# indrajeetadityaroy9/vit-inductive-bias-distillation

Hardware: AMD Instinct MI355X
Metric: distillation images/sec (BASD loss fwd+bwd+grad all-reduce), DeiT-S<-ResNet-50 @ bs256/GPU (higher is better)
Workload: dtype f32; 1 GPU; cfg2 DeiT-S<-ResNet-50 224x224; per_gpu_batch=256, global_batch=256, input_dtype=float32, layout=strided (CLS-sliced / channel-major views), backward=True, grad_allreduce_bytes=88202672, grad_allreduce=none at world size 1 (bucket packed, nothing to exchange), rank_readback=auto, readback_deferred_steps=1756, selector=basd_selector_chain mode 0, parallelism=dp1

## Files before the change

include/basd_hip.h:

```cpp
#ifndef BASD_HIP_H
#define BASD_HIP_H

#include <stdint.h>

#ifdef __cplusplus
extern "C" {
#endif

#ifndef __HIP_PLATFORM_AMD__
typedef struct ihipStream_t* hipStream_t;
#endif

#define BASD_OK 0
#define BASD_EINVAL (-1)
#define BASD_EUNSUPPORTED (-2)
#define BASD_DTYPE_F32 0
#define BASD_DTYPE_BF16 1


int basd_gemm_nt(const void* a, int a_dtype, long a_sb, long a_sn, long a_sd, int a_rows_per_batch,
                 long a_batch_stride, const float* b, long ldb, long b_batch_stride, int M, int N, int K, int batch,
                 float* c, long ldc, long c_batch_stride, float scale, const float* bias, float beta,
                 float* colsum_part, float* col_mean, hipStream_t stream);

// ... 144 lines not shown
                         const float* omega, const int* tap0, const int* tap1, const float* lam, const int* range0,
                         const int* range1, float* mu, float* tr_s, float* a_prime, hipStream_t stream);

int basd_teacher_center(const void* const* tok_ptrs, int dtype, const float* mix, int L, long sb, long sn, long sd,
                        int B, int n, int D, const int* g0, const int* g1, const float* glam, const float* omega_t,
                        float* mu, float* tc, hipStream_t stream);
int basd_teacher_center_multi(const void* const* tok_ptrs, int dtype, const float* mix, int L, int G, long sb, long sn,
                              long sd, int B, int n, int D, const int* g0, const int* g1, const float* glam,
                              const float* omega_t, float* mu, float* tc, hipStream_t stream);
long basd_teacher_center_stream_scratch_floats(int G, int B, int n, int D);
int basd_teacher_center_stream(const void* const* tok_ptrs, int dtype, const float* mix, int L, int G, long sb, long sn,
                               long sd, int B, int n, int D, const int* g0, const int* g1, const float* glam,
                               const float* omega_t, float* mu, float* tc, float* scratch, hipStream_t stream);

int basd_gram_f64(const float* p, long p_batch_stride, int n, int D, int batch, double* g, long g_batch_stride,
                  hipStream_t stream);

int basd_gram_f64_split(const float* p, long p_batch_stride, int n, int D, int batch, int splits, double* slabs,
                        double* g, hipStream_t stream);

int basd_chol_f64(const double* g, long g_batch_stride, int n, int batch, double* l, long l_batch_stride,
                  hipStream_t stream);

int basd_stack_product(const double* la, const double* lb, long l_batch_stride, int n, int batch, int lb_period,
                       float* w, long w_batch_stride, hipStream_t stream);

int basd_procrustes_finalize(const float* w, long w_batch_stride, const float* sigma, int n, int n_s, int batch,
                             int t_period ,
                             const double* gb, long g_batch_stride, const float* omega, const int* tap0,
                             const int* tap1, const float* lam, const float* tr_s_part, int tr_slabs, float* tr_s,
                             float* tr_t, float* nuc, float* loss, float* k_prime, hipStream_t stream);

int basd_student_grad(const void* x, int dtype, long sb, long sn, int B, int n_s, int n_t, int D, const float* omega,
                      const float* mu, const float* h, const int* tap0, const int* tap1, const float* lam,
                      const float* scale_ptr, float scale_const, float* dx, const float* tnorm2, float* gomega,
                      hipStream_t stream);

int basd_student_project_multi(const void* const* x_ptrs, int dtype, long sb, long sn, int E, int B, int n_s, int n_t,
                               int D, int ptrs_16B_aligned, const float* omega, long omega_e_stride, const int* tap0,
                               const int* tap1, const float* lam, const int* range0, const int* range1, float* mu,
                               float* tr_s, float* a_prime, hipStream_t stream);
int basd_student_grad_multi(const void* const* x_ptrs, int dtype, long sb, long sn, int E, int B, int n_s, int n_t,
                            int D, const float* omega, long omega_e_stride, const float* mu, const float* h,
                            const int* tap0, const int* tap1, const float* lam, const float* scale_ptr,
                            float scale_const, float* dx, const float* tnorm2, float* gomega, hipStream_t stream);
int basd_student_grad_fused(const void* const* x_ptrs, int dtype, long sb, long sn, int E, int B, int n_s, int n_t,
// ... 8 lines not shown
    long s_dtype, s_sb, s_sn, s_aligned;
    const void* const* tok_ptrs;
    long t_dtype, t_sb, t_sn, t_sd;
    const void* const* attn_ptrs;
    long a_dtype, a_sb, a_sh, a_sq, a_sk;
    const float* mix;
    long E, L, G, B, n_s, n_t, d_s, d_t, H, A, has_cls, n_a, n, max_sweeps;
    const int* atap0; const int* atap1; const float* alam;
    const int* tap0; const int* tap1; const float* lam; const int* range0; const int* range1;
    const int* g0; const int* g1; const float* glam;
    float* omega; float* omega_t; float* raw; float* mu_t; float* tc; float* mu_s; float* tr_part; float* tr_s;
    float* a_prime;
    double* g_all; double* l_all;
    float* W; float* sigma; int* jflags; int* sweeps;
    float* tr_t; float* nuc; float* loss_b; float* k_prime;
    float* h; float* dx; const float* grad_layers;
    double* g_slabs; long g_splits;
    const float* uw_ce; float* uw_out;
    void* jac_ws;
    float* w_stack; float* sigma_u;
} BasdProcrustesArgs;
int basd_procrustes_forward_fused(const BasdProcrustesArgs* args, hipStream_t stream);
int basd_procrustes_tuning(int transposed_cores);

int basd_stack_product_t(const double* la, const double* lb, long l_batch_stride, int n, int batch, int lb_period,
                         float* w, long w_batch_stride, hipStream_t stream);
int basd_kprime_from_transposed(const float* w, long w_batch_stride, const float* sigma, int n, int batch,
                                const double* lb, long l_batch_stride, int lb_period, float* z, long z_batch_stride,
                                float* k_prime, hipStream_t stream);
int basd_ustack_stash(const float* wc, long wc_batch_stride, int n, int batch, float* w_stack, long w_stack_stride,
                      hipStream_t stream);
int basd_ustack_from_transposed(const float* x, long x_batch_stride, const float* sigma, int n, int batch,
                                float* w_stack, long w_stack_stride, float* scratch, long scratch_batch_stride,
                                float* sigma_u, int max_sweeps, int* jflags, hipStream_t stream);

int basd_scale_unless_one(float* x, long count, const float* num, const float* den, hipStream_t stream);

int basd_cross_entropy(const void* logits, int dtype, long ld, int B, int C, const long* labels, const float* probs,
                       long pld, float label_smoothing, long ignore_index, float* row_loss, float* dlogits,
                       hipStream_t stream);


int basd_event_create(void** out);
int basd_event_destroy(void* event);
int basd_stream_wait_event(hipStream_t stream, void* event);
int basd_event_record(void* event, hipStream_t stream);
// ... 84 lines not shown
```

vit-inductive-bias-distillation_amd/basd_amd/_lib.py:

```python
from __future__ import annotations

import ctypes as C
import os
import threading

_HERE = os.path.dirname(os.path.abspath(__file__))
LIB_PATH = os.path.join(_HERE, "libbasd_hip.so")

vp, i32, i64, f32, f64 = C.c_void_p, C.c_int, C.c_long, C.c_float, C.c_double

SIGNATURES = {
    "basd_gemm_nt": [vp, i32, i64, i64, i64, i32, i64, vp, i64, i64, i32, i32, i32, i32, vp, i64, i64, f32, vp, f32,
                     vp, vp, vp],
    "basd_gemm_tn_splits": [i32],
    "basd_gemm_tn": [vp, vp, i32, i64, i64, i64, i64, i64, i64, i64, i64, i32, i32, i32, i32, i32, vp, vp, i32, vp,
                     vp, i64, i64, f32, vp],
    "basd_colmean_parts": [i32],
    "basd_colmean": [vp, i32, i64, i64, i64, i32, i64, i32, i32, i32, i32, vp, vp, vp],
    "basd_colmean_multi": [vp, i32, i64, i64, i64, i32, i32, i32, i32, i32, vp, vp, i32, vp],
    "basd_syrk_splits": [i32, i32, i32],
    "basd_syrk_multi": [vp, i32, i64, i64, i64, i32, i32, i32, i32, vp, vp, i32, vp, vp, i64, i32, vp, i32, i32, vp],
    "basd_jacobi_workspace_ints": [i32, i32],
    "basd_jacobi_twopass_workspace_bytes": [i32, i32, i32],
    "basd_jacobi_stacked_twopass": [vp, i64, i32, i32, vp, i32, i32, f32, vp, vp, vp],
# ... 16 lines not shown
    "basd_tridiag_eigenvalues": [vp, vp, i32, i32, vp, vp],
    "basd_tridiag_apply_q": [vp, vp, i32, i32, i32, vp, vp, i32, i32, vp],
    "basd_tridiag_shifted_solve": [vp, vp, vp, i32, i32, i32, i32, vp, vp, vp],
    "basd_tridiag_mp_rank": [vp, vp, i32, i32, f64, i32, vp, vp, vp, vp, vp],
    "basd_tridiag_mp_rank_rank1": [vp, vp, vp, i32, i32, f64, f64, i32, vp, vp, vp, vp],
    "basd_tridiag_eigenvectors": [vp, vp, vp, vp, vp, i32, i32, i32, vp, vp, i32, vp],
    "basd_mp_rank": [vp, i32, i32, f64, i32, vp, vp, vp],
    "basd_grassmann_distance": [vp, i32, vp, vp, i32, vp, i32, vp, vp, vp],
    "basd_grassmann_distance_padded": [vp, i32, i32, vp, vp, i32, vp, i32, vp, vp],
    "basd_selector_tail": [vp] * 10 + [i32, i32, i32, i32] + [vp] * 14 + [vp],
    "basd_sqrt_clamp": [vp, vp, i64, vp],
    "basd_gram_finish": [vp, vp, i32, i32, i64, vp, vp, vp],
    "basd_cross_entropy": [vp, i32, i64, i32, i32, vp, vp, i64, f32, i64, vp, vp, vp],
    "basd_token_weights": [vp, i32, vp, i32, i64, i64, i64, i64, i32, i32, i32, i32, i32, i32, i32, vp, vp, vp, vp,
                           vp, vp, vp, vp, vp, vp],
    "basd_student_project": [vp, i32, i64, i64, i32, i32, i32, i32, vp, vp, vp, vp, vp, vp, vp, vp, vp, vp],
    "basd_teacher_center": [vp, i32, vp, i32, i64, i64, i64, i32, i32, i32, vp, vp, vp, vp, vp, vp, vp],
    "basd_teacher_center_multi": [vp, i32, vp, i32, i32, i64, i64, i64, i32, i32, i32, vp, vp, vp, vp, vp, vp, vp],
    "basd_teacher_center_stream_scratch_floats": [i32, i32, i32, i32],
    "basd_teacher_center_stream": [vp, i32, vp, i32, i32, i64, i64, i64, i32, i32, i32, vp, vp, vp, vp, vp, vp, vp, vp],
    "basd_gram_f64": [vp, i64, i32, i32, i32, vp, i64, vp],
    "basd_gram_f64_split": [vp, i64, i32, i32, i32, i32, vp, vp, vp],
    "basd_chol_f64": [vp, i64, i32, i32, vp, i64, vp],
    "basd_stack_product": [vp, vp, i64, i32, i32, i32, vp, i64, vp],
    "basd_procrustes_finalize": [vp, i64, vp, i32, i32, i32, i32, vp, i64, vp, vp, vp, vp, vp, i32, vp, vp, vp, vp,
                                 vp, vp],
    "basd_student_project_multi": [vp, i32, i64, i64, i32, i32, i32, i32, i32, i32, vp, i64, vp, vp, vp, vp, vp, vp,
                                   vp, vp, vp],
    "basd_student_grad_multi": [vp, i32, i64, i64, i32, i32, i32, i32, i32, vp, i64, vp, vp, vp, vp, vp, vp, f32, vp,
                                vp, vp, vp],
    "basd_student_grad_fused": [vp, i32, i64, i64, i32, i32, i32, i32, i32, i32, vp, i64, vp, vp, vp, vp, vp, vp, vp,
                                f32, vp, vp],
    "basd_procrustes_forward_fused": [vp, vp],
    "basd_procrustes_tuning": [i32],
    "basd_jacobi_plain4_fits": [i32],
    "basd_stack_product_t": [vp, vp, i64, i32, i32, i32, vp, i64, vp],
    "basd_kprime_from_transposed": [vp, i64, vp, i32, i32, vp, i64, i32, vp, i64, vp, vp],
    "basd_ustack_stash": [vp, i64, i32, i32, vp, i64, vp],
    "basd_ustack_from_transposed": [vp, i64, vp, i32, i32, vp, i64, vp, i64, vp, i32, vp, vp],
    "basd_resample_tokens": [vp, i32, i64, i64, i64, i32, i32, i32, i32, vp, vp, vp, vp, vp],
    "basd_resample_tokens_adjoint": [vp, i32, i32, i32, i32, vp, vp, vp, vp, vp, vp, vp],
    "basd_student_grad": [vp, i32, i64, i64, i32, i32, i32, i32, vp, vp, vp, vp, vp, vp, vp, f32, vp, vp, vp, vp],
    "basd_teacher_factor": [vp, i64, vp, i32, i32, i32, vp, vp, i64, vp, vp, vp, vp, vp, vp, vp, vp, vp],
    "basd_teacher_factor_tiled": [vp, i64, vp, i32, i32, i32, vp, vp, i64, vp, vp, vp, vp, vp, vp, vp, vp, vp, vp],
    "basd_mix_grad_tokens": [vp, vp, i32, i32, i64, i64, i64, i32, i32, i32, i32, vp, vp, vp, vp, vp],
    "basd_mix_grad_tokens_scratch_floats": [i32, i32, i32, i32],
    "basd_mix_grad_tokens_onepass": [vp, vp, i32, i32, i64, i64, i64, i32, i32, i32, i32, vp, vp, vp, vp, vp, vp],
    "basd_token_weight_bwd": [vp, vp, i32, i32, i32, i32, vp, vp, vp, vp, vp, vp, i32, i32, i64, i64, i64, i64, i32,
                              i32, i32, vp, vp, vp],
    "basd_build_angle_stack": [vp, i32, vp, i32, vp, vp],
    "basd_grassmann_distance_bwd": [vp, vp, i32, vp, vp, i32, vp, vp, i32, vp, vp],
    "basd_eigvec_k2": [vp, vp, i32, i32, i32, vp, vp],
    "basd_selector_chain": [vp],
    "basd_rank_certificate": [vp, vp, i32, i32, f64, vp, vp, vp],
    "basd_rank_certificate_scratch_bytes": [i32],
    "basd_debug_fill_lds": [C.c_uint, vp],
    "basd_selector_chain_tail": [vp, i32, i32],
# ... 105 lines not shown
```

vit-inductive-bias-distillation_amd/basd_amd/ops.py:

```python
from __future__ import annotations

from dataclasses import dataclass
from functools import lru_cache

import torch

from . import _lib

import os

F32, BF16 = 0, 1
MAX_SWEEPS = 20
TWO_PASS_SVD = True
TRANSPOSED_MIX_GRAD = True
TWO_PASS_LOG_LIMIT = 16 << 30
EIG_SOLVER = os.environ.get("BASD_EIG_SOLVER", "tridiag")
if os.environ.get("BASD_GEMM_SPLIT") in ("0", "1"):
    _lib.call("basd_gemm_tuning", int(os.environ["BASD_GEMM_SPLIT"]))
if os.environ.get("BASD_JACOBI_ORDERING") in ("0", "1"):
    _lib.call("basd_jacobi_ordering", int(os.environ["BASD_JACOBI_ORDERING"]))


def _stream() -> int:
    return torch._C._cuda_getCurrentRawStream(torch._C._cuda_getDevice())


def _dtype_code(t: torch.Tensor) -> int:
    if t.dtype == torch.float32:
        return F32
    if t.dtype == torch.bfloat16:
        return BF16
    raise TypeError(f"unsupported dtype {t.dtype}")


def as_supported(t: torch.Tensor) -> torch.Tensor:
    if t.dtype in (torch.float32, torch.bfloat16):
        return t
# ... 472 lines not shown
        self.E, self.L, self.B, self.n_s, self.d_s, self.n_t, self.d_t = E, L, B, n_s, d_s, n_t, d_t
        n_a = A - (1 if has_cls else 0)
        n = min(n_s, n_t)
        self.n, self.n_a = n, n_a
        self.tp = taps(n_t, n_s, dev) if n_t < n_s else None
        self.gt = taps(n_t, n_s, dev) if n_t > n_s else None
        self.atp = taps(n_a, n_s, dev)
        G = self.G = 1 if L == 1 else E
        f32 = dict(device=dev, dtype=torch.float32)
        slabs = (d_s + 31) // 32
        EB, GB = E * B, G * B
        self.need_bwd, self.need_mix_grad, self.want_dx, self.want_uw = need_bwd, need_mix_grad, want_dx, want_uw
        self.kept_sizes = [G * B * n_s, E * B * d_s, EB * n * d_s, EB * n * n if need_bwd else 0, 4 * EB,
                           (4 + 2 * E) if want_uw else 0]
        self.kept_padded = [(c + 63) // 64 * 64 for c in self.kept_sizes]
        self.kept_total = sum(self.kept_padded)
        g_splits = 1
        if GB < 1024 and d_t >= 512:
            g_splits = max(1, min(1024 // GB, d_t // 256, 16))
        self.g_splits = g_splits
        self.g_all = torch.empty((EB + GB + (g_splits * GB if g_splits > 1 else 0), n, n), device=dev, dtype=torch.float64)
        self.l_all = torch.empty((EB + GB, n, n), device=dev, dtype=torch.float64)
        self.W = torch.empty((EB, n, 2 * n), **f32)
        self.tc = torch.empty((G, B, n, d_t), **f32)
        sizes = [GB * n, GB * d_t, EB * slabs, EB * n]
        padded = [(c + 63) // 64 * 64 for c in sizes]
        self.omega_t, self.mu_t, self.tr_part, self.sigma = (
            piece[:c] for piece, c in zip(torch.split(torch.empty((sum(padded),), **f32), padded), sizes))
        self.ints = torch.empty((_lib.query("basd_jacobi_workspace_ints", EB, MAX_SWEEPS) + EB,), device=dev,
                                dtype=torch.int32)
        self.sweeps = self.ints[-EB:] if want_sweeps else None
        transposed_mix = bool(need_mix_grad and need_bwd and _lib.query("basd_jacobi_plain4_fits", n)
                              and (EB >= 128 or TRANSPOSED_MIX_GRAD == "force") and TRANSPOSED_MIX_GRAD)
        jac_bytes = _lib.query("basd_jacobi_twopass_workspace_bytes", n, EB, MAX_SWEEPS) \
            if TWO_PASS_SVD and not transposed_mix else 0
        if jac_bytes > TWO_PASS_LOG_LIMIT or (jac_bytes > (256 << 20)
                                              and jac_bytes > torch.cuda.mem_get_info(dev)[0] // 2):
            jac_bytes = 0
        self.jac_ws = torch.empty((jac_bytes // 8 + 1,), device=dev, dtype=torch.int64) if jac_bytes > 0 else None
        self.h = torch.empty((E, B, n, d_s), **f32) if want_dx else None
        self.w_stack = None
        self.sigma_u = None
        if transposed_mix:
            self.w_stack = torch.empty((EB, n, 2 * n), **f32)
            self.sigma_u = torch.empty((EB, n), **f32)
        self.host_ptrs = (ctypes.c_void_p * E)()

        a = self.args = _lib.ProcrustesArgs()
        a.student_host_ptrs = ctypes.cast(self.host_ptrs, ctypes.c_void_p)
        (a.E, a.L, a.G, a.B, a.n_s, a.n_t, a.d_s, a.d_t, a.H, a.A, a.has_cls, a.n_a, a.n, a.max_sweeps) = \
            E, L, G, B, n_s, n_t, d_s, d_t, H, A, int(has_cls), n_a, n, MAX_SWEEPS
        if self.atp:
            a.atap0, a.atap1, a.alam = self.atp.tap0.data_ptr(), self.atp.tap1.data_ptr(), self.atp.lam.data_ptr()
        if self.tp:
            a.tap0, a.tap1, a.lam = self.tp.tap0.data_ptr(), self.tp.tap1.data_ptr(), self.tp.lam.data_ptr()
            a.range0, a.range1 = self.tp.range0.data_ptr(), self.tp.range1.data_ptr()
        if self.gt:
            a.g0, a.g1, a.glam = self.gt.tap0.data_ptr(), self.gt.tap1.data_ptr(), self.gt.lam.data_ptr()
        a.omega_t, a.mu_t, a.tc, a.tr_part = (self.omega_t.data_ptr(), self.mu_t.data_ptr(), self.tc.data_ptr(),
                                              self.tr_part.data_ptr())
        a.g_all, a.l_all, a.W = self.g_all.data_ptr(), self.l_all.data_ptr(), self.W.data_ptr()
        a.sigma, a.jflags, a.sweeps = self.sigma.data_ptr(), self.ints.data_ptr(), _ptr(self.sweeps)
        a.h = _ptr(self.h)
        a.g_slabs = self.g_all[EB + GB:].data_ptr() if g_splits > 1 else None
        a.g_splits = g_splits
        a.jac_ws = _ptr(self.jac_ws)
        a.w_stack = _ptr(self.w_stack)
        a.sigma_u = _ptr(self.sigma_u)


_PROCRUSTES_PLANS: dict = {}


def procrustes_forward(students: list[torch.Tensor], teachers: list[torch.Tensor], attns: list[torch.Tensor],
                       mix: torch.Tensor, has_cls: bool, *, need_backward: bool = True,
                       want_sweeps: bool = False, need_mix_grad: bool = False,
                       grad_layers: torch.Tensor | None = None,
                       uwso_ce: torch.Tensor | None = None) -> ProcrustesContext:
    import ctypes
    E, L = len(students), len(teachers)
    students = [as_supported(s) for s in students]
    students = _check_common_layout([s if s.stride(2) == 1 else s.contiguous() for s in students],
                                    "student token tensors")
    teachers = _check_common_layout([as_supported(t) for t in teachers], "teacher token tensors")
    attns = _check_common_layout([as_supported(a) for a in attns], "teacher attention tensors")
    _require_cuda(*students, *teachers, *attns, mix)
    s0, t0, a0 = students[0], teachers[0], attns[0]
    dev = s0.device
    B, n_s, d_s = s0.shape
    _, n_t, d_t = t0.shape
    H, A = a0.shape[1], a0.shape[2]
    need_bwd = need_backward or grad_layers is not None
    want_dx = grad_layers is not None or uwso_ce is not None
    stream = _stream()
# ... 188 lines not shown
```

vit-inductive-bias-distillation_amd/csrc/basd_common.h:

```cpp
#pragma once
#include <hip/hip_runtime.h>
#include <hip/hip_bf16.h>
#include <stdint.h>

#define BASD_OK 0
#define BASD_EINVAL (-1)
#define BASD_EUNSUPPORTED (-2)

#define BASD_DTYPE_F32 0
#define BASD_DTYPE_BF16 1

#define BASD_CHECK_ARG(cond) \
    do {                     \
        if (!(cond)) return BASD_EINVAL; \
    } while (0)

#define BASD_RETURN_LAST()                         \
    do {                                           \
        hipError_t e_ = hipGetLastError();         \
        return e_ == hipSuccess ? BASD_OK : (int)e_; \
    } while (0)

namespace basd {

constexpr int kWave = 64;

__device__ __forceinline__ float to_f32(float x) { return x; }
__device__ __forceinline__ float to_f32(__hip_bfloat16 x) { return __bfloat162float(x); }
#define BASD_GLOBAL_AS __attribute__((address_space(1)))
__device__ __forceinline__ float ldg_f32(const BASD_GLOBAL_AS float* p) { return *p; }
__device__ __forceinline__ float ldg_f32(const BASD_GLOBAL_AS __hip_bfloat16* p) {
    return __uint_as_float((unsigned)*(const BASD_GLOBAL_AS unsigned short*)p << 16);
}

template <typename T>
__device__ __forceinline__ T group_sum(T v, int width) {
    for (int m = width >> 1; m > 0; m >>= 1) v += __shfl_xor(v, m, width);
    return v;
}

template <int CTRL>
__device__ __forceinline__ float dpp_get(float x) {
    return __int_as_float(__builtin_amdgcn_update_dpp(0, __float_as_int(x), CTRL, 0xF, 0xF, true));
}
__device__ __forceinline__ float row16_allsum(float x) {
    x += dpp_get<0xB1>(x);
    x += dpp_get<0x4E>(x);
    x += dpp_get<0x141>(x);
// ... 52 lines not shown
```

vit-inductive-bias-distillation_amd/csrc/fused.hip:

```cpp
#include "basd_common.h"
#include "../../include/basd_hip.h"

namespace basd {

__global__ void __launch_bounds__(256) uwso_combine_kernel(const float* __restrict__ ce, const float* __restrict__ loss_b,
                                                           int E, int B, float* __restrict__ out) {
    constexpr int CH = 32;
    __shared__ double red[CH][4];
    const int tid = threadIdx.x;
    double geo_sum = 0.;
    for (int e0 = 0; e0 < E; e0 += CH) {
        const int ne = E - e0 < CH ? E - e0 : CH;
        for (int e = 0; e < ne; ++e) {
            double acc = 0.;
            for (int b = tid; b < B; b += 256) acc += (double)loss_b[(long)(e0 + e) * B + b];
            for (int m = 32; m > 0; m >>= 1) acc += __shfl_xor(acc, m, 64);
            if ((tid & 63) == 0) red[e][tid >> 6] = acc;
        }
        __syncthreads();
        if (tid == 0)
            for (int e = 0; e < ne; ++e) {
                const float layer = (float)(((red[e][0] + red[e][1]) + (red[e][2] + red[e][3])) / (double)B);
                out[4 + E + e0 + e] = layer;
                geo_sum += (double)layer;
// ... 82 lines not shown
    int rc;
#define BASD_TRY(call)            \
    do {                          \
        rc = (call);              \
        if (rc != BASD_OK) return rc; \
    } while (0)
    int centred = BASD_EUNSUPPORTED;
    for (int g = 0; g < G; ++g) {
        BASD_TRY(basd_token_weights(a->attn_ptrs, (int)a->a_dtype, a->mix + (long)g * L, L, a->a_sb, a->a_sh, a->a_sq,
                                    a->a_sk, B, H, A, (int)a->has_cls, n_a, n, n_s, a->atap0, a->atap1, a->alam,
                                    a->tap0, a->tap1, a->lam, a->omega + (long)g * B * n_s,
                                    a->omega_t + (long)g * B * n, a->raw ? a->raw + (long)g * B * n_a : nullptr, st));
    }
    if (G > 1 && L >= 4 && basd_teacher_center_stream_scratch_floats(G, B, n, d_t) <= (long)E * B * 2 * n * n) {
        centred = basd_teacher_center_stream(a->tok_ptrs, (int)a->t_dtype, a->mix, L, G, a->t_sb, a->t_sn, a->t_sd, B, n,
                                             d_t, a->g0, a->g1, a->glam, a->omega_t, a->mu_t, a->tc, a->W, st);
        if (centred != BASD_OK && centred != BASD_EUNSUPPORTED) return centred;
    }
    if (G > 1 && centred != BASD_OK) {
        centred = basd_teacher_center_multi(a->tok_ptrs, (int)a->t_dtype, a->mix, L, G, a->t_sb, a->t_sn, a->t_sd, B, n,
                                            d_t, a->g0, a->g1, a->glam, a->omega_t, a->mu_t, a->tc, st);
        if (centred != BASD_OK && centred != BASD_EUNSUPPORTED) return centred;
    }
    for (int g = 0; g < G && centred != BASD_OK; ++g) {
        BASD_TRY(basd_teacher_center(a->tok_ptrs, (int)a->t_dtype, a->mix + (long)g * L, L, a->t_sb, a->t_sn, a->t_sd,
                                     B, n, d_t, a->g0, a->g1, a->glam, a->omega_t + (long)g * B * n,
                                     a->mu_t + (long)g * B * d_t, a->tc + (long)g * B * n * d_t, st));
    }
    const long om_stride = G == 1 ? 0 : (long)B * n_s;
    int slabs = (d_s + 31) / 32;
    rc = basd_student_project_multi(a->student_ptrs, (int)a->s_dtype, a->s_sb, a->s_sn, E, B, n_s, n, d_s,
                                    (int)a->s_aligned, a->omega, om_stride, a->tap0, a->tap1, a->lam, a->range0,
                                    a->range1, a->mu_s, a->tr_part, a->a_prime, st);
    if (rc == BASD_EUNSUPPORTED) {
        slabs = (d_s + 63) / 64;
        for (int e = 0; e < E; ++e)
            BASD_TRY(basd_student_project(a->student_host_ptrs[e], (int)a->s_dtype, a->s_sb, a->s_sn, B, n_s, n, d_s,
                                          a->omega + e * om_stride, a->tap0, a->tap1, a->lam, a->range0, a->range1,
                                          a->mu_s + (long)e * B * d_s, a->tr_part + (long)e * B * slabs,
                                          a->a_prime + (long)e * B * n * d_s, st));
    } else if (rc != BASD_OK) {
        return rc;
    }
    const long nn = (long)n * n;
    const int EB = E * B, GB = G * B;
    BASD_TRY(basd_gram_f64(a->a_prime, (long)n * d_s, n, d_s, EB, a->g_all, nn, st));
    if (a->g_slabs && a->g_splits > 1)
        BASD_TRY(basd_gram_f64_split(a->tc, (long)n * d_t, n, d_t, GB, (int)a->g_splits, a->g_slabs,
                                     a->g_all + (long)EB * nn, st));
    else
        BASD_TRY(basd_gram_f64(a->tc, (long)n * d_t, n, d_t, GB, a->g_all + (long)EB * nn, nn, st));
    BASD_TRY(basd_chol_f64(a->g_all, nn, n, EB + GB, a->l_all, nn, st));
    if ((a->raw == nullptr || a->w_stack != nullptr) && EB <= 65535 && basd_jacobi_plain4_fits(n) &&
        (g_transposed_cores == 2 || (g_transposed_cores == 1 && EB >= 128))) {
        BASD_TRY(basd_stack_product_t(a->l_all, a->l_all + (long)EB * nn, nn, n, EB, GB, a->W, 2 * nn, st));
        if (a->raw != nullptr) BASD_TRY(basd_ustack_stash(a->W, 2 * nn, n, EB, a->w_stack, 2 * nn, st));
        BASD_TRY(basd_jacobi_onesided(a->W, 2 * nn, n, n, n, EB, nullptr, a->sigma, n, (int)a->max_sweeps, 0.f,
                                      a->jflags, a->sweeps, st));
        BASD_TRY(basd_procrustes_finalize(a->W, 2 * nn, a->sigma, n, n_s, EB, GB, a->g_all + (long)EB * nn, nn, a->omega,
                                          a->tap0, a->tap1, a->lam, a->tr_part, slabs, a->tr_s, a->tr_t, a->nuc,
                                          a->loss_b, nullptr, st));
        if (a->k_prime)
            BASD_TRY(basd_kprime_from_transposed(a->W, 2 * nn, a->sigma, n, EB, a->l_all + (long)EB * nn, nn, GB,
                                                 a->W + nn, 2 * nn, a->k_prime, st));
        if (a->raw != nullptr) {
            BASD_CHECK_ARG(a->sigma_u != nullptr);
            BASD_TRY(basd_ustack_from_transposed(a->W, 2 * nn, a->sigma, n, EB, a->w_stack, 2 * nn, a->W + nn, 2 * nn,
                                                 a->sigma_u, (int)a->max_sweeps, a->jflags, st));
        }
        return procrustes_tail(a, grad_layers_in, E, B, n_s, n, d_s, EB, nn, om_stride, st);
// ... 35 lines not shown
```

vit-inductive-bias-distillation_amd/csrc/procrustes.hip:

```cpp
#include "basd_common.h"
#include "../../include/basd_hip.h"

namespace basd {

typedef double f64x4 __attribute__((ext_vector_type(4)));

template <typename T>
__global__ void __launch_bounds__(256) token_weights_kernel(const void* const* __restrict__ attn_ptrs,
                                                            const float* __restrict__ mix, int L, long sb, long sh,
                                                            long sq, long sk, int H, int A, int has_cls, int n_a,
                                                            int n_t, int n_s, const int* __restrict__ atap0,
                                                            const int* __restrict__ atap1,
                                                            const float* __restrict__ alam,
                                                            const int* __restrict__ tap0,
                                                            const int* __restrict__ tap1,
                                                            const float* __restrict__ lam, float* __restrict__ omega,
                                                            float* __restrict__ omega_t, float* __restrict__ raw_out) {
    extern __shared__ float sm[];
    float* raw = sm;
    float* w = sm + n_a;
    __shared__ float red[32];
    const int b = blockIdx.x, tid = threadIdx.x;
    for (int j = tid; j < n_a; j += blockDim.x) {
        float acc = 0.f;
// ... 541 lines not shown
    double acc = 0.;
    for (int s2 = 0; s2 < splits; ++s2) acc += slabs[(long)s2 * split_stride + i];
    G[i] = acc;
}

static bool gram_f64_shape(int n, int* waves, int* chunks, size_t* lds) {
    const int nt = (n + 15) / 16, ntiles = nt * (nt + 1) / 2;
    int w = (ntiles + G64_TPW - 1) / G64_TPW;
    if (w < 4) w = ntiles < 4 ? ntiles : 4;
    int c = 1;
    if (w > 16) {
        c = (ntiles + 16 * G64_TPW - 1) / (16 * G64_TPW);
        w = 16;
    }
    *waves = w;
    *chunks = c;
    *lds = sizeof(float) * (size_t)nt * 16 * G64_LD;
    if (*lds > 156 * 1024) return false;
    if (*lds > 48 * 1024)
        (void)hipFuncSetAttribute((const void*)gram_f64_kernel, hipFuncAttributeMaxDynamicSharedMemorySize, 156 * 1024);
    return true;
}

__device__ __forceinline__ int pk(int i, int j, int n) { return j * n - (j * (j - 1)) / 2 + (i - j); }

__global__ void __launch_bounds__(1024) chol_f64_kernel(const double* __restrict__ G, long g_batch_stride, int n,
                                                        double* __restrict__ Lout, long l_batch_stride) {
    extern __shared__ __attribute__((aligned(16))) double a[];
    double* col = a + (size_t)n * (n + 1) / 2;
    __shared__ double sh_piv;
    __shared__ double red[32];
    const int m = blockIdx.x, tid = threadIdx.x, nthr = blockDim.x, lane = tid & 63, wave = tid >> 6, nw = nthr >> 6;
    const double* Gm = G + (long)m * g_batch_stride;
    double dmax = 0.;
    for (int j = wave; j < n; j += nw)
        for (int i = j + lane; i < n; i += 64) {
            const double v = Gm[(long)i * n + j];
            a[pk(i, j, n)] = v;
            if (i == j) dmax = fmax(dmax, v);
        }
    for (int s = 32; s > 0; s >>= 1) dmax = fmax(dmax, __shfl_xor(dmax, s, 64));
    if (lane == 0) red[wave] = dmax;
    __syncthreads();
    dmax = 0.;
    for (int i = 0; i < nw; ++i) dmax = fmax(dmax, red[i]);
    const double thr = dmax * (double)n * 1e-15;
// ... 319 lines not shown
    const int tx = tid & 31, ty = tid >> 5;
    float acc[4] = {0.f, 0.f, 0.f, 0.f};
    for (int c0 = 0; c0 < n; c0 += 32) {
        __syncthreads();
        for (int idx = tid; idx < 1024; idx += 256) {
            const int cc = idx >> 5, i = idx & 31, c = c0 + cc;
            za[cc][i] = (c < n && a0 + i < n) ? Zb[(long)c * n + a0 + i] : 0.f;
            zb[cc][i] = (c < n && b0 + i < n) ? Zb[(long)c * n + b0 + i] : 0.f;
        }
        __syncthreads();
#pragma unroll 8
        for (int cc = 0; cc < 32; ++cc) {
            const float bv = zb[cc][tx];
#pragma unroll
            for (int i = 0; i < 4; ++i) acc[i] = fmaf(za[cc][ty + 8 * i], bv, acc[i]);
        }
    }
    float* K = Kp + (long)b * n * n;
#pragma unroll
    for (int i = 0; i < 4; ++i) {
        const int a = a0 + ty + 8 * i, bb = b0 + tx;
        if (a < n && bb < n) K[(long)a * n + bb] = acc[i];
    }
}

__global__ void __launch_bounds__(256) procrustes_finalize_kernel(
    const float* __restrict__ W, long w_batch_stride, const float* __restrict__ sigma, int n, int n_s,
    const double* __restrict__ Gb, long g_batch_stride, const float* __restrict__ omega,
    const int* __restrict__ tap0, const int* __restrict__ tap1, const float* __restrict__ lam,
    const float* __restrict__ tr_s, int tr_slabs, float* __restrict__ tr_s_out, float* __restrict__ tr_t_out,
    float* __restrict__ nuc_out, float* __restrict__ loss_out, float* __restrict__ Kp, int t_period) {
    extern __shared__ float sm[];
    float* isig = sm;
    __shared__ float red[32];
    __shared__ double redd[32];
    const int b = blockIdx.x, tid = threadIdx.x;
    const float* sg = sigma + (long)b * n;
    float smax = 0.f, ssum = 0.f;
    for (int j = tid; j < n; j += 256) {
        smax = fmaxf(smax, sg[j]);
        ssum += sg[j];
    }
    smax = wave_max(smax);
    __syncthreads();
    if ((tid & 63) == 0) red[tid >> 6] = smax;
    __syncthreads();
// ... 218 lines not shown
}

__global__ void __launch_bounds__(128) resample_tokens_adjoint_kernel(const float* __restrict__ dY, int n_in,
                                                                      int n_out, int D,
                                                                      const int* __restrict__ tap0,
                                                                      const int* __restrict__ tap1,
                                                                      const float* __restrict__ lam,
                                                                      const int* __restrict__ range0,
                                                                      const int* __restrict__ range1,
                                                                      float* __restrict__ dX) {
    const int j = blockIdx.x, b = blockIdx.y;
    const int s0 = range0[j], s1 = range1[j];
    for (int d = threadIdx.x; d < D; d += 128) {
        float acc = 0.f;
        for (int s = s0; s < s1; ++s) {
            const float l1 = lam[s];
            const float coef = (tap0[s] == j ? 1.f - l1 : 0.f) + (tap1[s] == j ? l1 : 0.f);
            acc = fmaf(coef, dY[((long)b * n_out + s) * D + d], acc);
        }
        dX[((long)b * n_in + j) * D + d] = acc;
    }
}

}

using namespace basd;

extern "C" {

int basd_token_weights(const void* const* attn_ptrs, int dtype, const float* mix, int L, long sb, long sh, long sq,
                       long sk, int B, int H, int A, int has_cls, int n_a, int n_t, int n_s, const int* atap0,
                       const int* atap1, const float* alam, const int* tap0, const int* tap1, const float* lam,
                       float* omega, float* omega_t, float* raw_out, hipStream_t stream) {
    BASD_CHECK_ARG(attn_ptrs && mix && omega && omega_t && L > 0 && B > 0 && H > 0 && n_a > 0 && n_t > 0 && n_s > 0);
    BASD_CHECK_ARG(A == n_a + (has_cls ? 1 : 0));
    BASD_CHECK_ARG((n_a == n_s) == (atap0 == nullptr));
    BASD_CHECK_ARG((n_t == n_s) == (tap0 == nullptr));
    const size_t lds = sizeof(float) * (size_t)(n_a + n_s);
    if (dtype == BASD_DTYPE_F32)
        token_weights_kernel<float><<<B, 256, lds, stream>>>(attn_ptrs, mix, L, sb, sh, sq, sk, H, A, has_cls, n_a, n_t, n_s, atap0, atap1, alam, tap0, tap1, lam, omega, omega_t, raw_out);
    else if (dtype == BASD_DTYPE_BF16)
        token_weights_kernel<__hip_bfloat16><<<B, 256, lds, stream>>>(attn_ptrs, mix, L, sb, sh, sq, sk, H, A, has_cls, n_a, n_t, n_s, atap0, atap1, alam, tap0, tap1, lam, omega, omega_t, raw_out);
    else
        return BASD_EINVAL;
    BASD_RETURN_LAST();
}
// ... 179 lines not shown
                  hipStream_t stream) {
    BASD_CHECK_ARG(p && g && n > 0 && D > 0 && batch > 0);
    BASD_CHECK_ARG(((uintptr_t)p & 15) == 0 && D % 4 == 0 && p_batch_stride % 4 == 0);
    int waves, chunks;
    size_t lds;
    if (!gram_f64_shape(n, &waves, &chunks, &lds)) return BASD_EUNSUPPORTED;
    gram_f64_kernel<<<dim3(batch, 1, chunks), 64 * waves, lds, stream>>>(p, p_batch_stride, n, D, g, g_batch_stride, 0);
    BASD_RETURN_LAST();
}

int basd_gram_f64_split(const float* p, long p_batch_stride, int n, int D, int batch, int splits, double* slabs,
                        double* g, hipStream_t stream) {
    BASD_CHECK_ARG(p && g && slabs && n > 0 && D > 0 && batch > 0 && splits >= 1 && splits <= 64);
    BASD_CHECK_ARG(((uintptr_t)p & 15) == 0 && D % 4 == 0 && p_batch_stride % 4 == 0);
    int waves, chunks;
    size_t lds;
    if (!gram_f64_shape(n, &waves, &chunks, &lds)) return BASD_EUNSUPPORTED;
    const long count = (long)batch * n * n;
    gram_f64_kernel<<<dim3(batch, splits, chunks), 64 * waves, lds, stream>>>(p, p_batch_stride, n, D, slabs, (long)n * n, count);
    gram_f64_reduce_kernel<<<(unsigned)((count + 255) / 256), 256, 0, stream>>>(slabs, count, splits, count, g);
    BASD_RETURN_LAST();
}

int basd_chol_f64(const double* g, long g_batch_stride, int n, int batch, double* l, long l_batch_stride,
                  hipStream_t stream) {
    BASD_CHECK_ARG(g && l && n > 0 && batch > 0);
    const size_t lds = sizeof(double) * ((size_t)n * (n + 1) / 2 + n);
    if (lds > 158 * 1024) {
        if (n > 64 * CB_MAXR) return BASD_EUNSUPPORTED;
        const size_t lds_b = sizeof(double) * ((size_t)n * CB_NB + (size_t)CB_NB * (CB_KC + 1));
        (void)hipFuncSetAttribute((const void*)chol_f64_blocked_kernel, hipFuncAttributeMaxDynamicSharedMemorySize, 156 * 1024);
        chol_f64_blocked_kernel<<<batch, 1024, lds_b, stream>>>(g, g_batch_stride, n, l, l_batch_stride);
        BASD_RETURN_LAST();
    }
    (void)hipFuncSetAttribute((const void*)chol_f64_kernel, hipFuncAttributeMaxDynamicSharedMemorySize, 158 * 1024);
    const int threads = n >= 128 ? 1024 : n >= 64 ? 512 : 256;
    chol_f64_kernel<<<batch, threads, lds, stream>>>(g, g_batch_stride, n, l, l_batch_stride);
    BASD_RETURN_LAST();
}

int basd_stack_product(const double* la, const double* lb, long l_batch_stride, int n, int batch, int lb_period,
                       float* w, long w_batch_stride, hipStream_t stream) {
    BASD_CHECK_ARG(la && lb && w && n > 0 && batch > 0 && lb_period > 0);
    const size_t lds = sizeof(double) * 2 * (size_t)n * n;
    if (lds <= 78 * 1024) {
        (void)hipFuncSetAttribute((const void*)stack_product_kernel, hipFuncAttributeMaxDynamicSharedMemorySize, 78 * 1024);
        stack_product_kernel<<<batch, 256, lds, stream>>>(la, lb, l_batch_stride, n, w, w_batch_stride, lb_period);
    } else {
        BASD_CHECK_ARG(batch <= 65535);
        const int nt = (n + 31) / 32;
        stack_product_global_kernel<<<dim3(nt, nt, batch), 256, 0, stream>>>(la, lb, l_batch_stride, n, w, w_batch_stride, lb_period);
    }
    BASD_RETURN_LAST();
}

int basd_stack_product_t(const double* la, const double* lb, long l_batch_stride, int n, int batch, int lb_period,
                         float* w, long w_batch_stride, hipStream_t stream) {
    BASD_CHECK_ARG(la && lb && w && n > 0 && batch > 0 && lb_period > 0 && batch <= 65535);
    const int nt = (n + 31) / 32;
    stack_product_t_kernel<<<dim3(nt, nt, batch), 256, 0, stream>>>(la, lb, l_batch_stride, n, w, w_batch_stride, lb_period);
    BASD_RETURN_LAST();
}

int basd_kprime_from_transposed(const float* w, long w_batch_stride, const float* sigma, int n, int batch,
                                const double* lb, long l_batch_stride, int lb_period, float* z, long z_batch_stride,
                                float* k_prime, hipStream_t stream) {
    BASD_CHECK_ARG(w && sigma && lb && z && k_prime && n > 0 && batch > 0 && lb_period > 0 && batch <= 65535);
    const int nt = (n + 31) / 32;
    kprime_z_kernel<<<dim3(nt, nt, batch), 256, 0, stream>>>(w, w_batch_stride, sigma, n, lb, l_batch_stride, lb_period, z, z_batch_stride);
    kprime_from_z_kernel<<<dim3(nt, nt, batch), 256, 0, stream>>>(z, z_batch_stride, n, k_prime);
    BASD_RETURN_LAST();
}

int basd_ustack_stash(const float* wc, long wc_batch_stride, int n, int batch, float* w_stack, long w_stack_stride,
                      hipStream_t stream) {
    BASD_CHECK_ARG(wc && w_stack && n > 0 && batch > 0 && batch <= 65535 && w_stack_stride >= 2L * n * n);
    m_stash_kernel<<<dim3((unsigned)(((long)n * n + 255) / 256), batch), 256, 0, stream>>>(wc, wc_batch_stride, n, w_stack, w_stack_stride);
    BASD_RETURN_LAST();
}
int basd_ustack_from_transposed(const float* x, long x_batch_stride, const float* sigma, int n, int batch,
                                float* w_stack, long w_stack_stride, float* scratch, long scratch_batch_stride,
                                float* sigma_u, int max_sweeps, int* jflags, hipStream_t stream) {
    BASD_CHECK_ARG(x && sigma && w_stack && scratch && sigma_u && n > 0 && batch > 0 && batch <= 65535 &&
                   w_stack_stride >= 2L * n * n && scratch_batch_stride >= (long)n * n);
    const int nt = (n + 31) / 32;
    ustack_from_x_kernel<<<dim3(nt, nt, batch), 256, 0, stream>>>(x, x_batch_stride, sigma, n, w_stack, w_stack_stride, scratch, scratch_batch_stride);
    int rc = basd_jacobi_onesided(scratch, scratch_batch_stride, n, n, n, batch, nullptr, sigma_u, n, max_sweeps, 0.f,
                                  jflags, nullptr, stream);
    if (rc != BASD_OK) return rc;
    ustack_place_kernel<<<dim3((unsigned)(((long)n * n + 255) / 256), batch), 256, 0, stream>>>(scratch, scratch_batch_stride, n, w_stack, w_stack_stride);
// ... 140 lines not shown
```

Before: 161,700 images/s.

## Compute teacher Gram from raw tokens with algebraic centering; fuse k-prime kernels

When there is a single teacher layer and group, the teacher centering pass no longer writes a centered token copy. The Gram matrix is now built directly from raw tokens with f64 MFMA, then centered algebraically using omega weights (G - u_i - u_j + s), which removes a large intermediate write and read. Separately, for n<=64 the two k-prime kernels become one shared-memory kernel, saving a launch and a global round trip for z. A legacy-route toggle keeps the old path available. The risk is numerical differences from centering after accumulation rather than before.

```diff
diff --git a/include/basd_hip.h b/include/basd_hip.h
--- a/include/basd_hip.h
+++ b/include/basd_hip.h
@@ -190,6 +190,10 @@
 int basd_chol_f64(const double* g, long g_batch_stride, int n, int batch, double* l, long l_batch_stride,
                   hipStream_t stream);
 
+int basd_teacher_gram_centered(const void* const* tok_ptrs, int dtype, const float* mix, long sb, long sn, long sd, int B,
+                               int n, int D, const float* omega_t, int splits, double* slabs, double* g,
+                               hipStream_t stream);
+
 int basd_stack_product(const double* la, const double* lb, long l_batch_stride, int n, int batch, int lb_period,
                        float* w, long w_batch_stride, hipStream_t stream);
 
@@ -244,6 +248,7 @@
 } BasdProcrustesArgs;
 int basd_procrustes_forward_fused(const BasdProcrustesArgs* args, hipStream_t stream);
 int basd_procrustes_tuning(int transposed_cores);
+int basd_procrustes_legacy_route(int legacy);
 
 int basd_stack_product_t(const double* la, const double* lb, long l_batch_stride, int n, int batch, int lb_period,
                          float* w, long w_batch_stride, hipStream_t stream);
diff --git a/vit-inductive-bias-distillation_amd/basd_amd/_lib.py b/vit-inductive-bias-distillation_amd/basd_amd/_lib.py
--- a/vit-inductive-bias-distillation_amd/basd_amd/_lib.py
+++ b/vit-inductive-bias-distillation_amd/basd_amd/_lib.py
@@ -62,6 +62,7 @@
     "basd_gram_f64": [vp, i64, i32, i32, i32, vp, i64, vp],
     "basd_gram_f64_split": [vp, i64, i32, i32, i32, i32, vp, vp, vp],
     "basd_chol_f64": [vp, i64, i32, i32, vp, i64, vp],
+    "basd_teacher_gram_centered": [vp, i32, vp, i64, i64, i64, i32, i32, i32, vp, i32, vp, vp, vp],
     "basd_stack_product": [vp, vp, i64, i32, i32, i32, vp, i64, vp],
     "basd_procrustes_finalize": [vp, i64, vp, i32, i32, i32, i32, vp, i64, vp, vp, vp, vp, vp, i32, vp, vp, vp, vp,
                                  vp, vp],
@@ -73,6 +74,7 @@
                                 f32, vp, vp],
     "basd_procrustes_forward_fused": [vp, vp],
     "basd_procrustes_tuning": [i32],
+    "basd_procrustes_legacy_route": [i32],
     "basd_jacobi_plain4_fits": [i32],
     "basd_stack_product_t": [vp, vp, i64, i32, i32, i32, vp, i64, vp],
     "basd_kprime_from_transposed": [vp, i64, vp, i32, i32, vp, i64, i32, vp, i64, vp, vp],
diff --git a/vit-inductive-bias-distillation_amd/basd_amd/ops.py b/vit-inductive-bias-distillation_amd/basd_amd/ops.py
--- a/vit-inductive-bias-distillation_amd/basd_amd/ops.py
+++ b/vit-inductive-bias-distillation_amd/basd_amd/ops.py
@@ -13,6 +13,7 @@
 MAX_SWEEPS = 20
 TWO_PASS_SVD = True
 TRANSPOSED_MIX_GRAD = True
+LEGACY_ROUTE = False
 TWO_PASS_LOG_LIMIT = 16 << 30
 EIG_SOLVER = os.environ.get("BASD_EIG_SOLVER", "tridiag")
 if os.environ.get("BASD_GEMM_SPLIT") in ("0", "1"):
@@ -531,7 +532,8 @@
         self.g_all = torch.empty((EB + GB + (g_splits * GB if g_splits > 1 else 0), n, n), device=dev, dtype=torch.float64)
         self.l_all = torch.empty((EB + GB, n, n), device=dev, dtype=torch.float64)
         self.W = torch.empty((EB, n, 2 * n), **f32)
-        self.tc = torch.empty((G, B, n, d_t), **f32)
+        raw_gram = L == 1 and self.gt is None and not need_mix_grad and n <= 240 and not LEGACY_ROUTE
+        self.tc = None if raw_gram else torch.empty((G, B, n, d_t), **f32)
         sizes = [GB * n, GB * d_t, EB * slabs, EB * n]
         padded = [(c + 63) // 64 * 64 for c in sizes]
         self.omega_t, self.mu_t, self.tr_part, self.sigma = (
@@ -566,7 +568,7 @@
             a.range0, a.range1 = self.tp.range0.data_ptr(), self.tp.range1.data_ptr()
         if self.gt:
             a.g0, a.g1, a.glam = self.gt.tap0.data_ptr(), self.gt.tap1.data_ptr(), self.gt.lam.data_ptr()
-        a.omega_t, a.mu_t, a.tc, a.tr_part = (self.omega_t.data_ptr(), self.mu_t.data_ptr(), self.tc.data_ptr(),
+        a.omega_t, a.mu_t, a.tc, a.tr_part = (self.omega_t.data_ptr(), self.mu_t.data_ptr(), _ptr(self.tc),
                                               self.tr_part.data_ptr())
         a.g_all, a.l_all, a.W = self.g_all.data_ptr(), self.l_all.data_ptr(), self.W.data_ptr()
         a.sigma, a.jflags, a.sweeps = self.sigma.data_ptr(), self.ints.data_ptr(), _ptr(self.sweeps)
@@ -579,6 +581,15 @@
 
 
 _PROCRUSTES_PLANS: dict = {}
+
+
+def set_legacy_route(legacy: bool) -> None:
+    global LEGACY_ROUTE
+    if torch.cuda.is_available():
+        torch.cuda.synchronize()
+    _PROCRUSTES_PLANS.clear()
+    _lib.call("basd_procrustes_legacy_route", int(bool(legacy)))
+    LEGACY_ROUTE = bool(legacy)
 
 
 def procrustes_forward(students: list[torch.Tensor], teachers: list[torch.Tensor], attns: list[torch.Tensor],
diff --git a/vit-inductive-bias-distillation_amd/csrc/basd_common.h b/vit-inductive-bias-distillation_amd/csrc/basd_common.h
--- a/vit-inductive-bias-distillation_amd/csrc/basd_common.h
+++ b/vit-inductive-bias-distillation_amd/csrc/basd_common.h
@@ -24,6 +24,8 @@
 namespace basd {
 
 constexpr int kWave = 64;
+
+bool legacy_route();
 
 __device__ __forceinline__ float to_f32(float x) { return x; }
 __device__ __forceinline__ float to_f32(__hip_bfloat16 x) { return __bfloat162float(x); }
diff --git a/vit-inductive-bias-distillation_amd/csrc/fused.hip b/vit-inductive-bias-distillation_amd/csrc/fused.hip
--- a/vit-inductive-bias-distillation_amd/csrc/fused.hip
+++ b/vit-inductive-bias-distillation_amd/csrc/fused.hip
@@ -128,7 +128,8 @@
                                             d_t, a->g0, a->g1, a->glam, a->omega_t, a->mu_t, a->tc, st);
         if (centred != BASD_OK && centred != BASD_EUNSUPPORTED) return centred;
     }
-    for (int g = 0; g < G && centred != BASD_OK; ++g) {
+    const bool raw_gram = L == 1 && G == 1 && a->g0 == nullptr && a->raw == nullptr && n <= 240 && !basd::legacy_route();
+    for (int g = 0; g < G && centred != BASD_OK && !raw_gram; ++g) {
         BASD_TRY(basd_teacher_center(a->tok_ptrs, (int)a->t_dtype, a->mix + (long)g * L, L, a->t_sb, a->t_sn, a->t_sd,
                                      B, n, d_t, a->g0, a->g1, a->glam, a->omega_t + (long)g * B * n,
                                      a->mu_t + (long)g * B * d_t, a->tc + (long)g * B * n * d_t, st));
@@ -151,7 +152,11 @@
     const long nn = (long)n * n;
     const int EB = E * B, GB = G * B;
     BASD_TRY(basd_gram_f64(a->a_prime, (long)n * d_s, n, d_s, EB, a->g_all, nn, st));
-    if (a->g_slabs && a->g_splits > 1)
+    if (raw_gram)
+        BASD_TRY(basd_teacher_gram_centered(a->tok_ptrs, (int)a->t_dtype, a->mix, a->t_sb, a->t_sn, a->t_sd, B, n, d_t,
+                                            a->omega_t, a->g_slabs && a->g_splits > 1 ? (int)a->g_splits : 1,
+                                            a->g_slabs, a->g_all + (long)EB * nn, st));
+    else if (a->g_slabs && a->g_splits > 1)
         BASD_TRY(basd_gram_f64_split(a->tc, (long)n * d_t, n, d_t, GB, (int)a->g_splits, a->g_slabs,
                                      a->g_all + (long)EB * nn, st));
     else
diff --git a/vit-inductive-bias-distillation_amd/csrc/procrustes.hip b/vit-inductive-bias-distillation_amd/csrc/procrustes.hip
--- a/vit-inductive-bias-distillation_amd/csrc/procrustes.hip
+++ b/vit-inductive-bias-distillation_amd/csrc/procrustes.hip
@@ -587,6 +587,106 @@
     return true;
 }
 
+template <typename T>
+__global__ void __launch_bounds__(1024) teacher_gram_raw_kernel(const void* const* __restrict__ tok_ptrs, long sb,
+                                                                long sn, long sd, int n, int D,
+                                                                double* __restrict__ G, long g_split_stride) {
+    extern __shared__ __attribute__((aligned(16))) float tile[];
+    const int b = blockIdx.x, tid = threadIdx.x, lane = tid & 63, wave = tid >> 6, nw = blockDim.x >> 6;
+    G += (long)blockIdx.y * g_split_stride;
+    const int nt = (n + 15) / 16, ntiles = nt * (nt + 1) / 2;
+    const BASD_GLOBAL_AS T* Pb = (const BASD_GLOBAL_AS T*)tok_ptrs[0] + (long)b * sb;
+    f64x4 acc[G64_TPW];
+#pragma unroll
+    for (int t = 0; t < G64_TPW; ++t) acc[t] = f64x4{0., 0., 0., 0.};
+    int ti[G64_TPW], tj[G64_TPW];
+#pragma unroll
+    for (int t = 0; t < G64_TPW; ++t) {
+        const int lin = wave + t * nw;
+        int r = 0;
+        if (lin < ntiles) {
+            r = (int)((sqrtf(8.f * lin + 1.f) - 1.f) * 0.5f);
+            while ((r + 1) * (r + 2) / 2 <= lin) ++r;
+            while (r * (r + 1) / 2 > lin) --r;
+            ti[t] = r;
+            tj[t] = lin - r * (r + 1) / 2;
+        } else {
+            ti[t] = -1;
+            tj[t] = -1;
+        }
+    }
+    for (int idx = n * G64_LD + tid; idx < nt * 16 * G64_LD; idx += blockDim.x) tile[idx] = 0.f;
+    const bool feat_fast = sd == 1;
+    const int i16 = lane & 15, kq = lane >> 4;
+    for (int k0 = blockIdx.y * G64_BK; k0 < D; k0 += G64_BK * gridDim.y) {
+        __syncthreads();
+        for (int idx = tid; idx < n * G64_BK; idx += blockDim.x) {
+            int r, c;
+            if (feat_fast) { r = idx / G64_BK; c = idx - r * G64_BK; }
+            else { c = idx / n; r = idx - c * n; }
+            const int k = k0 + c;
+            tile[r * G64_LD + c] = k < D ? ldg_f32(Pb + ((long)r * sn + (long)k * sd)) : 0.f;
+        }
+        __syncthreads();
+#pragma unroll
+        for (int g = 0; g < G64_BK / 16; ++g) {
+#pragma unroll
+            for (int t = 0; t < G64_TPW; ++t) {
+                if (ti[t] < 0) continue;
+                const float4 a = *(const float4*)(tile + (ti[t] * 16 + i16) * G64_LD + g * 16 + 4 * kq);
+                const float4 bb = *(const float4*)(tile + (tj[t] * 16 + i16) * G64_LD + g * 16 + 4 * kq);
+                acc[t] = __builtin_amdgcn_mfma_f64_16x16x4f64((double)a.x, (double)bb.x, acc[t], 0, 0, 0);
+                acc[t] = __builtin_amdgcn_mfma_f64_16x16x4f64((double)a.y, (double)bb.y, acc[t], 0, 0, 0);
+                acc[t] = __builtin_amdgcn_mfma_f64_16x16x4f64((double)a.z, (double)bb.z, acc[t], 0, 0, 0);
+                acc[t] = __builtin_amdgcn_mfma_f64_16x16x4f64((double)a.w, (double)bb.w, acc[t], 0, 0, 0);
+            }
+        }
+    }
+    double* Gb = G + (long)b * n * n;
+#pragma unroll
+    for (int t = 0; t < G64_TPW; ++t) {
+        if (ti[t] < 0) continue;
+        const int col = tj[t] * 16 + (lane & 15);
+#pragma unroll
+        for (int r = 0; r < 4; ++r) {
+            const int row = ti[t] * 16 + (lane >> 4) + 4 * r;
+            if (row < n && col < n) {
+                Gb[(long)row * n + col] = acc[t][r];
+                Gb[(long)col * n + row] = acc[t][r];
+            }
+        }
+    }
+}
+
+__global__ void __launch_bounds__(256) teacher_gram_center_kernel(const double* slabs, long split_stride, int splits,
+                                                                  int n, const float* __restrict__ mix,
+                                                                  const float* __restrict__ omega_t, double* G) {
+    __shared__ double w[256], u[256], red[32];
+    const int b = blockIdx.x, tid = threadIdx.x, nn = n * n;
+    const double* Sb = slabs + (long)b * nn;
+    double* Gb = G + (long)b * nn;
+    const double m2 = mix ? (double)mix[0] * (double)mix[0] : 1.;
+    if (tid < n) w[tid] = (double)omega_t[(long)b * n + tid];
+    for (int idx = tid; idx < nn; idx += 256) {
+        double acc = 0.;
+        for (int s2 = 0; s2 < splits; ++s2) acc += Sb[(long)s2 * split_stride + idx];
+        Gb[idx] = acc * m2;
+    }
+    __syncthreads();
+    double su = 0.;
+    if (tid < n) {
+        double acc = 0.;
+        for (int j = 0; j < n; ++j) acc = fma(Gb[(long)j * n + tid], w[j], acc);
+        u[tid] = acc;
+        su = w[tid] * acc;
+    }
+    const double s = block_sum(su, red);
+    for (int idx = tid; idx < nn; idx += 256) {
+        const int i = idx / n, j = idx - i * n;
+        Gb[idx] = (Gb[idx] - (u[i] + u[j])) + s;
+    }
+}
+
 __device__ __forceinline__ int pk(int i, int j, int n) { return j * n - (j * (j - 1)) / 2 + (i - j); }
 
 __global__ void __launch_bounds__(1024) chol_f64_kernel(const double* __restrict__ G, long g_batch_stride, int n,
@@ -952,6 +1052,90 @@
         const int a = a0 + ty + 8 * i, bb = b0 + tx;
         if (a < n && bb < n) K[(long)a * n + bb] = acc[i];
     }
+}
+
+constexpr int KF_N = 64, KF_LD = KF_N + 1;
+__global__ void __launch_bounds__(256) kprime_fused_kernel(const float* __restrict__ W, long w_batch_stride,
+                                                           const float* __restrict__ sigma, int n,
+                                                           const double* __restrict__ Lb, long l_batch_stride,
+                                                           int lb_period, float* __restrict__ Kp) {
+    extern __shared__ float kf_sm[];
+    float* xs = kf_sm;
+    float* ls = xs + n * KF_LD;
+    float* zs = ls + n * KF_LD;
+    __shared__ float red[4];
+    const int b = blockIdx.x, tid = threadIdx.x;
+    const float* sg = sigma + (long)b * n;
+    float smax = 0.f;
+    for (int j = tid; j < n; j += 256) smax = fmaxf(smax, sg[j]);
+    smax = wave_max(smax);
+    if ((tid & 63) == 0) red[tid >> 6] = smax;
+    const float* Wb = W + (long)b * w_batch_stride;
+    const double* L = Lb + (long)(b % lb_period) * l_batch_stride;
+    for (int idx = tid; idx < n * n; idx += 256) {
+        const int q = idx / n, r = idx - q * n;
+        xs[q * KF_LD + r] = Wb[idx];
+        ls[q * KF_LD + r] = r <= q ? (float)L[idx] : 0.f;
+    }
+    __syncthreads();
+    smax = fmaxf(fmaxf(red[0], red[1]), fmaxf(red[2], red[3]));
+    const float thr = smax * (float)n * 1.1920929e-7f;
+    const int tx = tid & 15, ty = tid >> 4;
+    int ra[4], rc[4];
+#pragma unroll
+    for (int i = 0; i < 4; ++i) {
+        ra[i] = min(tx + 16 * i, n - 1) * KF_LD;
+        rc[i] = min(ty + 16 * i, n - 1) * KF_LD;
+    }
+    float acc[4][4];
+#pragma unroll
+    for (int q = 0; q < 4; ++q)
+#pragma unroll
+        for (int i = 0; i < 4; ++i) acc[q][i] = 0.f;
+    for (int r = 0; r < n; ++r) {
+        float lv[4], xv[4];
+#pragma unroll
+        for (int i = 0; i < 4; ++i) lv[i] = ls[ra[i] + r];
+#pragma unroll
+        for (int q = 0; q < 4; ++q) xv[q] = xs[rc[q] + r];
+#pragma unroll
+        for (int q = 0; q < 4; ++q)
+#pragma unroll
+            for (int i = 0; i < 4; ++i) acc[q][i] = fmaf(lv[i], xv[q], acc[q][i]);
+    }
+#pragma unroll
+    for (int q = 0; q < 4; ++q) {
+        const int c = ty + 16 * q;
+        if (c >= n) continue;
+        const float sv = sg[c];
+        const float sc = sv > thr ? 1.f / (sv * sqrtf(sv)) : 0.f;
+#pragma unroll
+        for (int i = 0; i < 4; ++i) zs[c * KF_LD + tx + 16 * i] = acc[q][i] * sc;
+    }
+    __syncthreads();
+#pragma unroll
+    for (int q = 0; q < 4; ++q)
+#pragma unroll
+        for (int i = 0; i < 4; ++i) acc[q][i] = 0.f;
+    for (int c = 0; c < n; ++c) {
+        float av[4], bv[4];
+#pragma unroll
+        for (int q = 0; q < 4; ++q) av[q] = zs[c * KF_LD + ty + 16 * q];
+#pragma unroll
+        for (int i = 0; i < 4; ++i) bv[i] = zs[c * KF_LD + tx + 16 * i];
+#pragma unroll
+        for (int q = 0; q < 4; ++q)
+#pragma unroll
+            for (int i = 0; i < 4; ++i) acc[q][i] = fmaf(av[q], bv[i], acc[q][i]);
+    }
+    float* K = Kp + (long)b * n * n;
+#pragma unroll
+    for (int q = 0; q < 4; ++q)
+#pragma unroll
+        for (int i = 0; i < 4; ++i) {
+            const int a = ty + 16 * q, bb = tx + 16 * i;
+            if (a < n && bb < n) K[(long)a * n + bb] = acc[q][i];
+        }
 }
 
 __global__ void __launch_bounds__(256) procrustes_finalize_kernel(
@@ -1216,6 +1400,9 @@
     }
 }
 
+static int g_legacy_route = 0;
+bool legacy_route() { return g_legacy_route != 0; }
+
 }
 
 using namespace basd;
@@ -1441,6 +1628,31 @@
     BASD_RETURN_LAST();
 }
 
+int basd_procrustes_legacy_route(int legacy) {
+    if (legacy >= 0) g_legacy_route = legacy != 0;
+    return BASD_OK;
+}
+
+int basd_teacher_gram_centered(const void* const* tok_ptrs, int dtype, const float* mix, long sb, long sn, long sd, int B,
+                               int n, int D, const float* omega_t, int splits, double* slabs, double* g,
+                               hipStream_t stream) {
+    BASD_CHECK_ARG(tok_ptrs && omega_t && g && B > 0 && n > 0 && D > 0 && splits >= 1 && splits <= 64);
+    BASD_CHECK_ARG(splits == 1 || slabs != nullptr);
+    BASD_CHECK_ARG(dtype == BASD_DTYPE_F32 || dtype == BASD_DTYPE_BF16);
+    int waves, chunks;
+    size_t lds;
+    if (!gram_f64_shape(n, &waves, &chunks, &lds) || chunks != 1) return BASD_EUNSUPPORTED;
+    const long count = (long)B * n * n;
+    double* part = splits > 1 ? slabs : g;
+    const dim3 grid(B, splits);
+    if (dtype == BASD_DTYPE_F32)
+        teacher_gram_raw_kernel<float><<<grid, 64 * waves, lds, stream>>>(tok_ptrs, sb, sn, sd, n, D, part, count);
+    else
+        teacher_gram_raw_kernel<__hip_bfloat16><<<grid, 64 * waves, lds, stream>>>(tok_ptrs, sb, sn, sd, n, D, part, count);
+    teacher_gram_center_kernel<<<B, 256, 0, stream>>>(part, count, splits, n, mix, omega_t, g);
+    BASD_RETURN_LAST();
+}
+
 int basd_chol_f64(const double* g, long g_batch_stride, int n, int batch, double* l, long l_batch_stride,
                   hipStream_t stream) {
     BASD_CHECK_ARG(g && l && n > 0 && batch > 0);
@@ -1485,6 +1697,13 @@
                                 const double* lb, long l_batch_stride, int lb_period, float* z, long z_batch_stride,
                                 float* k_prime, hipStream_t stream) {
     BASD_CHECK_ARG(w && sigma && lb && z && k_prime && n > 0 && batch > 0 && lb_period > 0 && batch <= 65535);
+    if (n <= KF_N && !g_legacy_route) {
+        const size_t lds = sizeof(float) * 3 * (size_t)n * KF_LD;
+        if (lds > 48 * 1024)
+            (void)hipFuncSetAttribute((const void*)kprime_fused_kernel, hipFuncAttributeMaxDynamicSharedMemorySize, 64 * 1024);
+        kprime_fused_kernel<<<batch, 256, lds, stream>>>(w, w_batch_stride, sigma, n, lb, l_batch_stride, lb_period, k_prime);
+        BASD_RETURN_LAST();
+    }
     const int nt = (n + 31) / 32;
     kprime_z_kernel<<<dim3(nt, nt, batch), 256, 0, stream>>>(w, w_batch_stride, sigma, n, lb, l_batch_stride, lb_period, z, z_batch_stride);
     kprime_from_z_kernel<<<dim3(nt, nt, batch), 256, 0, stream>>>(z, z_batch_stride, n, k_prime);
```

Result: slower. 159,900 images/s (-1.1%).
